# usnistgov/thermoextrap

Measured on AMD Instinct MI355X. Metric: samples/s for order-4 comoment bootstrap (N_samp x N_obs x nrep resample_vals), higher is better.
Workload: dtype f64; 1 GPU; north: central-comoment bootstrap, N_samp=1e+08, N_obs=32, order=4, nrep=1000, exact multinomial device sampler; n_samp=100000000, n_obs=32, order=4, nrep=1000, parallelism=state-points x1

## Files before the change

thermoextrap_amd/csrc/txm_i8g.h:

```cpp
#pragma once
#include "txm_i8t_common.h"

namespace txm {

constexpr int G_REPS = 128;
constexpr int G_KSTEP_BYTES = 32 * G_REPS;
constexpr int G_TILE_BYTES = SM_T * G_REPS;

static inline size_t count_table_bytes(int64_t ntiles, int64_t nreps) {
  return (size_t)cdiv(nreps, G_REPS) * (size_t)ntiles * G_TILE_BYTES;
}

constexpr int G_BS = 4;
constexpr int G_RAW = 2 * G_BS * 256;
#ifndef TXM_G_LEAD
#define TXM_G_LEAD 2
#endif
constexpr uint32_t G_LEAD = TXM_G_LEAD;

__device__ __forceinline__ void g_dma16(const void *sbase, uint32_t voff, uint32_t lds_dst) {
#ifdef TXM_G_NO_DMA
  return;
#endif
  asm volatile("s_mov_b32 m0, %2\n\ts_nop 0\n\tglobal_load_lds_dwordx4 %1, %0" ::"s"(sbase), "v"(voff), "s"(lds_dst) : "memory", "m0");
}
__device__ __forceinline__ void g_dma16_stream(const void *sbase, uint32_t voff, uint32_t lds_dst) {
#ifdef TXM_G_NO_DMA
  return;
#endif
#ifdef TXM_G_TABLE_PLAIN
  asm volatile("s_mov_b32 m0, %2\n\ts_nop 0\n\tglobal_load_lds_dwordx4 %1, %0" ::"s"(sbase), "v"(voff), "s"(lds_dst) : "memory", "m0");
#else
  asm volatile("s_mov_b32 m0, %2\n\ts_nop 0\n\tglobal_load_lds_dwordx4 %1, %0 nt" ::"s"(sbase), "v"(voff), "s"(lds_dst) : "memory", "m0");
#endif
}
__device__ __forceinline__ void g_dma4(const void *sbase, uint32_t voff, uint32_t lds_dst) {
#ifdef TXM_G_NO_DMA
  return;
#endif
  asm volatile("s_mov_b32 m0, %2\n\ts_nop 0\n\tglobal_load_lds_dword %1, %0" ::"s"(sbase), "v"(voff), "s"(lds_dst) : "memory", "m0");
}
__device__ __forceinline__ void g_load16(v4i &dst, const void *sbase, uint32_t voff) {
  asm volatile("global_load_dwordx4 %0, %1, %2" : "=v"(dst) : "v"(voff), "s"(sbase) : "memory");
}
typedef uint32_t g_v16u __attribute__((ext_vector_type(16)));
__device__ __forceinline__ uint32_t g_min_progress(const uint32_t *pg) {
  g_v16u v;
  asm volatile("s_load_dwordx16 %0, %1, 0x0 glc\n\ts_waitcnt lgkmcnt(0)" : "=s"(v) : "s"(pg) : "memory");
  uint32_t m = 0xffffffffu;
#pragma unroll
  for (int i = 0; i < 16; ++i) {
    const uint32_t e = v[i] == 0u ? 0xffffffffu : v[i];
    m = e < m ? e : m;
  }
  return m;
}
__device__ __forceinline__ uint32_t g_lane_now() {
  uint32_t l;
  asm volatile("v_mbcnt_lo_u32_b32 %0, -1, 0\n\tv_mbcnt_hi_u32_b32 %0, -1, %0" : "=v"(l));
  return l;
}
template <int N>
__device__ __forceinline__ void g_wait_vm() {
  asm volatile("s_waitcnt vmcnt(%0)" ::"n"(N) : "memory");
}


int launch_count_table(const uint32_t *counts, int64_t nrep, int64_t N, uint32_t k0, uint32_t k1, uint32_t rep_base,
                       int64_t rep_begin, int64_t n_groups, unsigned char *table, hipStream_t st);

bool i8g_applicable(const double *x, int64_t ldx_s, int64_t C, const double *y, int64_t ldy_s);
int launch_resample_i8g(const I8Args &a, int K, bool weighted, const unsigned char *table, int64_t rep_begin, int n_grp,
                        hipStream_t st);

bool i8gn_applicable(const double *x, int64_t ldx_s, int64_t C, int K);
int launch_resample_i8gn(const I8Args &a, int K, bool weighted, const unsigned char *table, int64_t rep_begin, int n_grp,
                         size_t table_state_stride, hipStream_t st);

}
```

thermoextrap_amd/csrc/txm_resample_i8g.hip:

```cpp
#include "txm_i8g.h"

namespace txm {

constexpr int G_XR = 4;
static_assert(G_XR == G_BS && G_BS == 4, "the wait counts below are written for blocks of four k-steps");
constexpr int G_XRB = 8;
constexpr int G_FU = 2176;

#ifdef TXM_G_FOUR_QUARTERS
template <int NS> constexpr int G_QUARTERS = 4;
#elif defined(TXM_G_SIX_QUARTERS)
template <int NS> constexpr int G_QUARTERS = NS == 1 ? 8 : NS == 2 ? 6 : 4;
#else
template <int NS> constexpr int G_QUARTERS = NS == 1 ? 8 : 4;
#endif

template <int J0, int JN, bool WEIGHTED, bool YS>
constexpr int G_NQ = (J0 == 0 && JN == 1 && WEIGHTED && YS) ? 4 : G_QUARTERS<JN + (YS ? 1 : 0)>;

template <int J0, int JN, bool WEIGHTED, bool YS>
__global__ __launch_bounds__(T_BLOCK) __attribute__((amdgpu_waves_per_eu(2, 2))) void resample_i8g_kernel(
    const I8Args a, const int K, const unsigned char *__restrict__ table, const int64_t rep_begin, const int n_grp) {
  constexpr int NS = JN + (YS ? 1 : 0);
  static_assert(JN >= 1 && NS <= 3 && J0 + JN <= 8, "row sets");
  constexpr int NPT = JN + ((YS && WEIGHTED && J0 > 0) ? 1 : 0);
  constexpr int NX = YS ? 2 : 1;
  constexpr int WREG = NS * T_PB;
  constexpr int NQ = G_NQ<J0, JN, WEIGHTED, YS>;
  constexpr int A_STEP = NQ * 1024;
  constexpr int PPW = G_BS * NQ / T_WAVES;
  static_assert(G_BS * NQ % T_WAVES == 0, "count pieces per wave");
  constexpr int OFF_A = T_WAVES * WREG;
  constexpr bool XBLK = !YS;
#ifdef TXM_G_ADIR
  constexpr bool ADIR = XBLK && NS == 2;
#else
  constexpr bool ADIR = false;
#endif
  constexpr int XRN = XBLK ? G_XRB : G_XR;
  constexpr int OFF_X = OFF_A + 2 * G_BS * A_STEP;
  constexpr int OFF_Y = OFF_X + T_WAVES * XRN * 1024;
  constexpr int OFF_RAW = OFF_Y + (YS ? T_WAVES * XRN * 1024 : 0);
  constexpr int OFF_F = OFF_RAW + 3 * G_RAW;
  constexpr int OFF_FS = OFF_F + 3 * 2 * G_FU;
  static_assert(G_BS * 16 * NPT * 8 <= G_FU, "factor lines");
  extern __shared__ __attribute__((aligned(16))) unsigned char lds[];
  uint32_t *fsum = reinterpret_cast<uint32_t *>(lds + OFF_FS);

  const int wave = __builtin_amdgcn_readfirstlane((int)(threadIdx.x >> 6)), lane = threadIdx.x & 63;
  const int n32 = lane & 31, half = lane >> 5;
  const uint32_t wreg = (uint32_t)(wave * WREG);

  const int b = blockIdx.x;
  const int n_wgg = (4 * n_grp + NQ - 1) / NQ;
  const int64_t win = (int64_t)((b >> 3) / n_wgg) * 8 + (b & 7);
  const int grp = (b >> 3) % n_wgg;
  if (win >= a.nwin) return;
  if (a.wflag[win] != 0u) return;
  const int64_t rep0 = rep_begin + (int64_t)grp * (32 * NQ);
  const int64_t WT = a.win_tiles;
  const int64_t t0 = win * WT;
  const int64_t t1 = t0 + WT < a.ntiles ? t0 + WT : a.ntiles;
  const int nsteps = (int)(t1 - t0) * T_STEPS;
  const int nblk = nsteps / G_BS;
  const unsigned char *tab = table + (size_t)t0 * G_TILE_BYTES;
  auto q_off = [&](int Q) -> size_t {
    int gq = grp * NQ + Q;
    if (gq >= 4 * n_grp) gq = grp * NQ;
    return (size_t)(gq >> 2) * (size_t)a.ntiles * G_TILE_BYTES + (size_t)(gq & 3) * 1024;
  };

  const int ps = lane >> 2, cl = lane & 3;
  const int col = 4 * wave + cl;
  const int ccol = col < a.C ? col : 0;
  const int qsrc = 4 * wave < a.C ? wave : 0;
  const uint32_t rd_off = wreg + (uint32_t)(((lane >> 4) & 1) * (T_PLANE + 128) + (16 * half + ((lane & 15) >> 1)) * 16 + (lane & 1) * 8);
  const int tcl = (n32 >> 2) & 3, tdg = 4 * (n32 >> 4) + (n32 & 3);
  const int ofi = wave >> 1;
  const int odig = 4 * (wave & 1) + cl;
  const uint32_t osel = odig < 7 ? (((uint32_t)odig << 24) | 0x000c0c0cu) : 0x0c0c0c0cu;
  const uint32_t oxor = odig < 6 ? 0x80000000u : 0u;

  const double *wt = a.wtab + win * I8_WT_STRIDE;
  const double pu = a.pivot[0];
  const double inv_du = wt[I8_WT_INVDU];
  const double inv_w = WEIGHTED ? wt[I8_WT_INVW] : 1.0;
  const double sc = wt[I8_WT_SC + ccol];
  const double px = a.pivot[1 + a.col0 + ccol];
  const double *wty = YS ? a.ywtab + win * I8_WT_STRIDE : wt;
  const double scy = YS ? wty[I8_WT_SC + ccol] : 0.0;
  const double py = YS ? a.ypivot[1 + a.col0 + ccol] : 0.0;

  v16i acc[NS][NQ];
#pragma unroll
  for (int e = 0; e < NS; ++e)
#pragma unroll
    for (int q = 0; q < NQ; ++q) acc[e][q] = (v16i)(0);

#ifdef TXM_G_CLOCKS
  const long long gc0 = clock64(), gr0 = wall_clock64();
#endif
#ifdef TXM_G_TIMING
  long long tm[8] = {0, 0, 0, 0, 0, 0, 0, 0};
  long long tk0 = clock64();
#define G_TICK(k) do { const long long t1_ = clock64(); tm[k] += t1_ - tk0; tk0 = t1_; } while (0)
#else
#define G_TICK(k) do {} while (0)
#endif
  auto chunk_sample = [&](int c) -> int64_t {
    int64_t b0 = (t0 + (c >> 5)) * SM_T;
    if (b0 > a.N - SM_T) b0 = a.N - SM_T;
    return b0 + 32 * (c & 31);
  };
  const uint32_t xring = (uint32_t)(OFF_X + wave * XRN * 1024), yring = (uint32_t)(OFF_Y + wave * XRN * 1024);
  int cq = 0;
  const char *xq = reinterpret_cast<const char *>(a.x + chunk_sample(0) * a.ldx_s);
  const char *yq = YS ? reinterpret_cast<const char *>(a.y + chunk_sample(0) * a.ldy_s) : nullptr;
  const int64_t xstep = 32 * a.ldx_s * 8, ystep = YS ? 32 * a.ldy_s * 8 : 0;
  const bool loader = !XBLK || wave < 4;
  const int qsrc2 = 4 * (wave + 4) < a.C ? wave + 4 : 0;
  const int64_t xcol1 = (a.col0 + 4 * qsrc) * 8, xcol2 = (a.col0 + 4 * qsrc2) * 8;
  size_t qoff[NQ];
#pragma unroll
  for (int Q = 0; Q < NQ; ++Q) qoff[Q] = q_off(Q);
  auto x_request = [&](int slot) {
#ifdef TXM_G_NO_XDMA
    if (slot >= 0) { ++cq; return; }
#endif
    if constexpr (XBLK) {
      if (loader) {
        const uint32_t ln = g_lane_now();
        const uint32_t row = (ln >> 1) * (uint32_t)(a.ldx_s * 8) + (ln & 1) * 16u + (uint32_t)(a.col0 * 8);
        g_dma16(xq, row + (uint32_t)(32 * qsrc), xring + (uint32_t)slot * 1024u);
        g_dma16(xq, row + (uint32_t)(32 * qsrc2), xring + (uint32_t)(4 * XRN * 1024) + (uint32_t)slot * 1024u);
      }
    } else {
      const uint32_t ln = g_lane_now();
      const uint32_t cb = (ln & 1) * 16u + (uint32_t)((a.col0 + 4 * qsrc) * 8);
      g_dma16(xq, (ln >> 1) * (uint32_t)(a.ldx_s * 8) + cb, xring + (uint32_t)slot * 1024u);
      if constexpr (YS) g_dma16(yq, (ln >> 1) * (uint32_t)(a.ldy_s * 8) + cb, yring + (uint32_t)slot * 1024u);
    }
    ++cq;
    if (cq < nsteps) {
      if ((cq & 31) == 0) {
        const int64_t i0 = chunk_sample(cq);
        xq = reinterpret_cast<const char *>(a.x + i0 * a.ldx_s);
        if constexpr (YS) yq = reinterpret_cast<const char *>(a.y + i0 * a.ldy_s);
      } else {
        xq += xstep;
        if constexpr (YS) yq += ystep;
      }
    }
  };
  auto a_request = [&](int B, int piece = -1) {
    const int Bc = B < nblk ? B : nblk - 1;
#ifdef TXM_G_NO_ADMA
    if (Bc >= 0) return;
#endif
    if constexpr (XBLK) {
      if (!loader) return;
      const unsigned char *src = tab + (size_t)(Bc * G_BS + wave) * G_KSTEP_BYTES;
      const uint32_t dst = (uint32_t)(OFF_A + (B & 1) * (G_BS * A_STEP) + wave * A_STEP);
#pragma unroll
      for (int Q = 0; Q < NQ; ++Q)
        if (piece < 0 || piece == Q) g_dma16_stream(src + q_off(Q), g_lane_now() * 16u, dst + (uint32_t)(Q * 1024));
    } else {
      const uint32_t l16 = g_lane_now() * 16u;
#pragma unroll
      for (int k = 0; k < PPW; ++k) {
        const int i = wave * PPW + k, st = i / NQ, Q = i % NQ;
        g_dma16_stream(tab + (size_t)(Bc * G_BS + st) * G_KSTEP_BYTES + q_off(Q), l16,
                (uint32_t)(OFF_A + (B & 1) * (G_BS * A_STEP) + st * A_STEP + Q * 1024));
      }
    }
  };
  auto raw_request = [&](int B) {
    int c = B * G_BS + 1 + (wave & 3);
    if (c > nsteps - 1) c = nsteps - 1;
    if constexpr (XBLK) {
      if (!loader) return;
      const int64_t i0 = chunk_sample(c);
      const uint32_t l4 = g_lane_now() * 4u;
      g_dma4(a.u + i0, l4, (uint32_t)(OFF_RAW + (B % 3) * G_RAW + wave * 256));
      if constexpr (WEIGHTED) g_dma4(a.w + i0, l4, (uint32_t)(OFF_RAW + (B % 3) * G_RAW + G_BS * 256 + wave * 256));
    } else {
      const double *src = ((WEIGHTED && wave >= 4) ? a.w : a.u) + chunk_sample(c);
      g_dma4(src, g_lane_now() * 4u, (uint32_t)(OFF_RAW + (B % 3) * G_RAW + (wave >> 2) * (G_BS * 256) + (wave & 3) * 256));
    }
  };
  auto stage_factors = [&](int B) {
#ifndef TXM_G_SW
#define TXM_G_SW 6
#endif
    constexpr int SW = TXM_G_SW;
    if (wave < SW || wave >= SW + 2) return;
    const int e = (int)g_lane_now() + (wave - SW) * 64;
    const double *raw = reinterpret_cast<const double *>(lds + OFF_RAW + (B % 3) * G_RAW);
#ifdef TXM_G_TIMING
    G_TICK(1);
    double r0 = raw[e];
    asm volatile("s_waitcnt lgkmcnt(0)" : "+v"(r0));
    G_TICK(5);
    const double du = (r0 - pu) * inv_du;
#else
    const double du = (raw[e] - pu) * inv_du;
#endif
    double pw = WEIGHTED ? raw[G_BS * 32 + e] * inv_w : 1.0;
    double *f = reinterpret_cast<double *>(lds + OFF_F + (B % 3) * (2 * G_FU) + ((e >> 4) & 1) * G_FU) + (((e >> 5) * 16 + (e & 15)) * NPT);
    if constexpr (NPT > JN) f[JN] = pw;
#pragma unroll
    for (int k = 0; k < J0; ++k) pw *= du;
#pragma unroll
    for (int jj = 0; jj < JN; ++jj) {
      if (WEIGHTED || J0 + jj > 0) f[jj] = pw;
      pw *= du;
    }
  };

  auto store_x2 = [&](uint32_t lo0, uint32_t hi0, uint32_t lo1, uint32_t hi1, int off) {
#ifdef TXM_G_PLAIN_STORES
    typedef __attribute__((address_space(3))) uint32_t *lds_u32;
    const uint32_t base = wreg + g_lane_now() * 4u;
    *(lds_u32)(lds + base + off) = lo0;
    *(lds_u32)(lds + base + off + T_PLANE + 128) = hi0;
    *(lds_u32)(lds + base + off + 256) = lo1;
    *(lds_u32)(lds + base + off + 256 + T_PLANE + 128) = hi1;
    return;
#endif
#ifdef TXM_G_PLAIN_STORES_ASM
    {
      const uint32_t base = wreg + g_lane_now() * 4u + (uint32_t)off;
      asm volatile("ds_write2st64_b32 %0, %1, %2 offset0:0 offset1:1\n\t"
                   "ds_write2st64_b32 %3, %4, %5 offset0:0 offset1:1"
                   :
                   : "v"(base), "v"(lo0), "v"(lo1), "v"(base + (uint32_t)(T_PLANE + 128)), "v"(hi0), "v"(hi1)
                   : "memory");
      return;
    }
#endif
    asm volatile("s_mov_b32 m0, %4\n\ts_nop 0\n\t"
                 "ds_write_addtid_b32 %0 offset:%5\n\t"
                 "ds_write_addtid_b32 %1 offset:%6\n\t"
                 "ds_write_addtid_b32 %2 offset:%7\n\t"
                 "ds_write_addtid_b32 %3 offset:%8"
                 :
                 : "v"(lo0), "v"(hi0), "v"(lo1), "v"(hi1), "s"(wreg), "n"(off), "n"(off + T_PLANE + 128), "n"(off + 256),
                   "n"(off + 256 + T_PLANE + 128)
                 : "memory", "m0");
  };
  auto produce_row = [&](auto fic, double (&f)[2], const double (&d)[2], auto &&ahead) {
    constexpr int fi = decltype(fic)::value;
    uint32_t lo[2], hi[2];
#pragma unroll
    for (int uu = 0; uu < 2; ++uu) {
      const uint64_t bits = (uint64_t)__double_as_longlong(fma(f[uu], d[uu], T_MAGIC));
      lo[uu] = (uint32_t)bits ^ 0x80808080u;
      hi[uu] = (uint32_t)(bits >> 32) ^ 0x00008080u;
    }
#ifdef TXM_G_NO_OVERLAY
    if (false) {
#else
    if (fi < JN && ofi == fi) {
#endif
#pragma unroll
      for (int uu = 0; uu < 2; ++uu) {
        const uint64_t ub = (uint64_t)__double_as_longlong(__builtin_ldexp(f[uu], 50) + T_MAGIC);
        uint32_t dig;
        asm volatile("v_perm_b32 %0, %1, %2, %3" : "=v"(dig) : "v"((uint32_t)(ub >> 32)), "v"((uint32_t)ub), "v"(osel));
        hi[uu] = (hi[uu] & 0x00ffffffu) | (dig ^ oxor);
      }
    }
    ahead();
    store_x2(lo[0], hi[0], lo[1], hi[1], fi * T_PB);
  };

  typedef __attribute__((address_space(3))) const double *lds_cd;
  typedef __attribute__((address_space(3))) const v4i *lds_cv4;

  if (threadIdx.x < 32 * NQ) {
    const int64_t r = rep0 + threadIdx.x;
    uint32_t s = 0;
    if (r < a.nrep)
      for (int64_t t = t0; t < t1; ++t) s += a.counts[(size_t)r * a.ntiles + t];
    fsum[threadIdx.x] = s;
  }
  for (int e = threadIdx.x; e < T_WAVES * WREG / 16; e += T_BLOCK) reinterpret_cast<uint4 *>(lds)[e] = make_uint4(0, 0, 0, 0);
  double d_du[2], d_w[2] = {1.0, 1.0};
  {
    const int64_t i0 = chunk_sample(0);
#pragma unroll
    for (int uu = 0; uu < 2; ++uu) {
      d_du[uu] = (a.u[i0 + 16 * uu + ps] - pu) * inv_du;
      if constexpr (WEIGHTED) d_w[uu] = a.w[i0 + 16 * uu + ps] * inv_w;
    }
  }
  asm volatile("s_waitcnt vmcnt(0)" ::: "memory");
  raw_request(0);
  raw_request(1);
  if constexpr (!ADIR) a_request(0);
  if constexpr (XBLK) {
    x_request(7);
#pragma unroll
    for (int c = 0; c < G_BS; ++c) x_request(c);
  } else {
#pragma unroll
    for (int c = 0; c < G_XR; ++c) x_request(c);
  }
  v4i AD[
#ifdef TXM_G_ADIR
      (XBLK && NS == 2) ? G_BS : 1
#else
      1
#endif
  ][NQ];
#ifdef TXM_G_ADIR
  if constexpr (XBLK && NS == 2) {
    const uint32_t l16 = g_lane_now() * 16u;
#pragma unroll
    for (int pp = 0; pp < G_BS; ++pp)
#pragma unroll
      for (int q = 0; q < NQ; ++q) g_load16(AD[pp][q], tab + (size_t)pp * G_KSTEP_BYTES + qoff[q], l16);
  }
#endif
  asm volatile("s_waitcnt vmcnt(0) lgkmcnt(0)\n\ts_barrier" ::: "memory");
  stage_factors(0);
  {
    const uint32_t xa = xring + (uint32_t)(ps * 32 + cl * 8) + (XBLK ? 7u * 1024u : 0u);
    double dx[2], dy[2] = {0.0, 0.0};
#pragma unroll
    for (int uu = 0; uu < 2; ++uu) {
      dx[uu] = (*(lds_cd)(lds + xa + uu * 512) - px) * sc;
      if constexpr (YS) dy[uu] = (*(lds_cd)(lds + xa + (yring - xring) + uu * 512) - py) * scy;
    }
    t_static_for<NS>([&](auto fic) {
      constexpr int fi = decltype(fic)::value;
      double f[2];
#pragma unroll
      for (int uu = 0; uu < 2; ++uu) {
        if constexpr (YS && fi == JN) {
          f[uu] = WEIGHTED ? d_w[uu] : 1.0;
        } else {
          double pw = WEIGHTED ? d_w[uu] : 1.0;
          for (int q = 0; q < J0 + fi; ++q) pw *= d_du[uu];
          f[uu] = pw;
        }
      }
      if constexpr (YS && fi == JN) produce_row(fic, f, dy, [] {});
      else produce_row(fic, f, dx, [] {});
    });
  }
  asm volatile("s_waitcnt lgkmcnt(0)\n\ts_barrier" ::: "memory");
  if constexpr (!XBLK) x_request(0);
  G_TICK(0);

  uint32_t *pg = a.progress != nullptr ? a.progress + (size_t)win * 16 : nullptr;
#ifdef TXM_G_PRIO
  if (wave >= 4) __builtin_amdgcn_s_setprio(TXM_G_PRIO);
#endif
  auto read_factors = [&](auto pnc, auto finc, uint32_t fb, double (&f)[2]) {
    constexpr int pn = decltype(pnc)::value, fin = decltype(finc)::value;
#pragma unroll
    for (int uu = 0; uu < 2; ++uu) {
      if constexpr (YS && fin == JN) {
        if constexpr (WEIGHTED) f[uu] = *(lds_cd)(lds + fb + uu * G_FU + (pn * 16 * NPT + (J0 == 0 ? 0 : JN)) * 8);
        else f[uu] = 1.0;
      } else if constexpr (!WEIGHTED && J0 == 0 && fin == 0) {
        f[uu] = 1.0;
      } else {
        f[uu] = *(lds_cd)(lds + fb + uu * G_FU + (pn * 16 * NPT + fin) * 8);
      }
    }
  };
  v4i A[NQ];
  constexpr bool BT2 = NS >= 2;
  v2i Bt[BT2 ? 2 : 1][2];
  double f[2], xr[2], yr[2] = {0.0, 0.0};
  uint32_t f_va = (uint32_t)(OFF_F + ps * NPT * 8);
  uint32_t x_va = xring + (uint32_t)(ps * 32 + cl * 8);
  {
    const uint32_t a_va0 = (uint32_t)OFF_A + (uint32_t)lane * 16u;
#pragma unroll
    for (int q = 0; q < NQ; ++q) {
      if constexpr (!ADIR) A[q] = *(lds_cv4)(lds + a_va0 + q * 1024);
    }
    Bt[0][0] = T_TRREAD((lds_v2i)(lds + rd_off));
    Bt[0][1] = T_TRREAD((lds_v2i)(lds + rd_off + 128));
    read_factors(std::integral_constant<int, 0>{}, std::integral_constant<int, 0>{}, f_va, f);
#pragma unroll
    for (int uu = 0; uu < 2; ++uu) xr[uu] = *(lds_cd)(lds + x_va + (XBLK ? 0 : 1024) + uu * 512);
  }
#pragma unroll 1
  for (int B = 0; B < nblk; ++B) {
    if (pg != nullptr && wave == 0 && (B & 7) == 0) {
      const uint32_t done = (uint32_t)(B >> 3) + 1u;
      if (lane == 0) __hip_atomic_store(&pg[grp & 15], done, __ATOMIC_RELAXED, __HIP_MEMORY_SCOPE_AGENT);
#pragma unroll 1
      for (int spin = 0; spin < I8_THROTTLE_SPINS; ++spin) {
        if (done <= g_min_progress(pg) + G_LEAD) break;
        __builtin_amdgcn_s_sleep(32);
      }
    }
    G_TICK(1);
    stage_factors(B + 1);
    G_TICK(7);
    raw_request(B + 2);
    const unsigned char *blk_asrc = nullptr;
    uint32_t blk_adst = 0, blk_l16 = 0, blk_xrow = 0;
    if constexpr (XBLK) {
      if (loader) {
        const int Bn = B + 1 < nblk ? B + 1 : nblk - 1;
        blk_asrc = tab + (size_t)(Bn * G_BS + wave) * G_KSTEP_BYTES;
        blk_adst = (uint32_t)(OFF_A + ((B + 1) & 1) * (G_BS * A_STEP) + wave * A_STEP);
        const uint32_t ln = g_lane_now();
        blk_l16 = ln * 16u;
        blk_xrow = (ln >> 1) * (uint32_t)(a.ldx_s * 8) + (ln & 1) * 16u;
      }
    }
    auto a_piece = [&](int Q) {
#ifndef TXM_G_NO_ADMA
      if constexpr (!ADIR)
        if (loader) g_dma16_stream(blk_asrc + qoff[Q], blk_l16, blk_adst + (uint32_t)(Q * 1024));
#endif
    };
    const unsigned char *nb_src = nullptr;
    uint32_t nb_l16 = 0;
    if constexpr (ADIR) {
      const int Bn = B + 1 < nblk ? B + 1 : nblk - 1;
      nb_src = tab + (size_t)(Bn * G_BS) * G_KSTEP_BYTES;
      nb_l16 = g_lane_now() * 16u;
    }
    auto x_chunk = [&](int i) {
#ifndef TXM_G_NO_XDMA
      if (loader) {
        const uint32_t dst = xring + (uint32_t)((4 * ((B + 1) & 1) + i) * 1024);
        g_dma16(xq + xcol1, blk_xrow, dst);
        g_dma16(xq + xcol2, blk_xrow, dst + (uint32_t)(4 * XRN * 1024));
      }
#endif
      ++cq;
      if (cq < nsteps) {
        if ((cq & 31) == 0) xq = reinterpret_cast<const char *>(a.x + chunk_sample(cq) * a.ldx_s);
        else xq += xstep;
      }
    };
#ifdef TXM_G_BURST
    constexpr bool SPREAD = false;
#else
    constexpr bool SPREAD = XBLK && NS >= 2;
#endif
    if constexpr (!SPREAD) {
      if constexpr (XBLK) {
#pragma unroll
        for (int Q = 0; Q < NQ; ++Q) a_piece(Q);
#pragma unroll
        for (int i = 0; i < G_BS; ++i) x_chunk(i);
      } else {
        a_request(B + 1);
      }
    }
    constexpr int ISSUE_SLOTS = 2 * NS;
    auto issue_items = [&](auto kc) {
      constexpr int k = decltype(kc)::value;
      if constexpr (SPREAD && k < ISSUE_SLOTS) {
        if constexpr (ADIR) {
          static_assert(!ADIR || ISSUE_SLOTS == G_BS, "one x chunk a slot");
          x_chunk(k);
        } else {
#pragma unroll
          for (int j = 0; j < NQ + 4; ++j)
            if (j * ISSUE_SLOTS / (NQ + 4) == k) {
              if (j < 8 && (j & 1) == 0) a_piece(j >> 1);
              else if (j < 8) x_chunk(j >> 1);
              else a_piece(j - 4);
            }
        }
      }
    };
    G_TICK(2);
    uint32_t a_va = (uint32_t)(OFF_A + (B & 1) * (G_BS * A_STEP)) + (uint32_t)lane * 16u;
    asm volatile("" : "+v"(f_va), "+v"(x_va), "+v"(a_va));
#ifdef TXM_G_NO_PIN
#define G_PIN() do {} while (0)
#else
#define G_PIN() __builtin_amdgcn_sched_barrier(0)
#endif
    t_static_for<G_BS>([&](auto pc) {
      constexpr int p = decltype(pc)::value;
      double dx[2], dy[2] = {0.0, 0.0};
      if constexpr (ADIR) {
        constexpr int R = WEIGHTED ? 2 : 1;
        constexpr int NL = 12 + (p < 2 ? 4 : 8) + R;
        G_PIN();
        if (loader) asm volatile("s_waitcnt vmcnt(%0)" ::"n"(NL) : "memory");
        else asm volatile("s_waitcnt vmcnt(12)" ::: "memory");
        G_PIN();
      }
      t_static_for<NS>([&](auto fic) {
        constexpr int fi = decltype(fic)::value;
        constexpr bool last = fi == NS - 1;
        if constexpr (p == G_BS - 1 && last) {
          G_TICK(3);
          if constexpr (ADIR) {
            if (loader) asm volatile("s_waitcnt vmcnt(7) lgkmcnt(0)" ::: "memory");
            else asm volatile("s_waitcnt lgkmcnt(0)" ::: "memory");
          } else {
            asm volatile("s_waitcnt vmcnt(%0) lgkmcnt(0)" ::"n"(XBLK ? 0 : 3 * NX) : "memory");
          }
#ifndef TXM_G_NO_BARRIER
          asm volatile("s_barrier" ::: "memory");
#endif
          G_TICK(6);
        }
        auto ahead = [&]() {
          if constexpr (!last) {
            read_factors(pc, std::integral_constant<int, fi + 1>{}, f_va, f);
          } else if constexpr (p < G_BS - 1) {
            read_factors(std::integral_constant<int, p + 1>{}, std::integral_constant<int, 0>{}, f_va, f);
          } else {
            f_va = (uint32_t)(OFF_F + ((B + 1) % 3) * (2 * G_FU) + ps * NPT * 8);
            asm volatile("" : "+v"(f_va));
            read_factors(std::integral_constant<int, 0>{}, std::integral_constant<int, 0>{}, f_va, f);
          }
          if constexpr (YS && fi == JN - 1) {
#pragma unroll
            for (int uu = 0; uu < 2; ++uu) yr[uu] = *(lds_cd)(lds + x_va + (OFF_Y - OFF_X) + ((p + 1) & 3) * 1024 + uu * 512);
          }
          if constexpr (last) {
            if constexpr (XBLK) {
              if constexpr (p == G_BS - 1) {
                x_va = xring + (uint32_t)(ps * 32 + cl * 8) + (uint32_t)(((B + 1) & 1) * 4096);
                asm volatile("" : "+v"(x_va));
              }
#pragma unroll
              for (int uu = 0; uu < 2; ++uu) xr[uu] = *(lds_cd)(lds + x_va + (p == G_BS - 1 ? 0 : p + 1) * 1024 + uu * 512);
            } else {
              g_wait_vm<2 * NX + (p == G_BS - 1 ? 0 : PPW + 1)>();
#pragma unroll
              for (int uu = 0; uu < 2; ++uu) xr[uu] = *(lds_cd)(lds + x_va + ((p + 2) & 3) * 1024 + uu * 512);
            }
          }
        };
        constexpr int bcur = BT2 ? ((p * NS + fi) & 1) : 0;
        const v4i Bv = {Bt[bcur][0][0], Bt[bcur][0][1], Bt[bcur][1][0], Bt[bcur][1][1]};
        auto mfma_q = [&](auto qc) {
          constexpr int q = decltype(qc)::value;
          if constexpr (ADIR) t_mfma<true>(acc[fi][q], AD[p][q], Bv);
          else t_mfma<true>(acc[fi][q], A[q], Bv);
#ifndef TXM_G_NO_AREAD
          if constexpr (last && ADIR) {
            g_load16(AD[p][q], nb_src + (size_t)p * G_KSTEP_BYTES + qoff[q], nb_l16);
          } else if constexpr (last) {
            if constexpr (p == G_BS - 1) {
              const uint32_t a_vn = (uint32_t)(OFF_A + ((B + 1) & 1) * (G_BS * A_STEP)) + g_lane_now() * 16u;
              A[q] = *(lds_cv4)(lds + a_vn + q * 1024);
            } else {
              A[q] = *(lds_cv4)(lds + a_va + (p + 1) * A_STEP + q * 1024);
            }
          }
#endif
        };
        G_PIN();
        t_static_for<(0 + 1) * NQ / 4 - 0 * NQ / 4>([&](auto jc) { mfma_q(std::integral_constant<int, 0 * NQ / 4 + decltype(jc)::value>{}); });
        G_PIN();
        issue_items(std::integral_constant<int, p * NS + fi>{});
        if constexpr (BT2) {
          constexpr int fn = (fi + 1) % NS;
          Bt[bcur ^ 1][0] = T_TRREAD((lds_v2i)(lds + rd_off + fn * T_PB));
          Bt[bcur ^ 1][1] = T_TRREAD((lds_v2i)(lds + rd_off + fn * T_PB + 128));
        }
        G_PIN();
        if constexpr (fi == 0) {
#pragma unroll
          for (int uu = 0; uu < 2; ++uu) dx[uu] = (xr[uu] - px) * sc;
        }
        if constexpr (YS && fi == JN) {
#pragma unroll
          for (int uu = 0; uu < 2; ++uu) dy[uu] = (yr[uu] - py) * scy;
        }
        uint32_t lo[2], hi[2];
#pragma unroll
        for (int uu = 0; uu < 2; ++uu) {
#ifdef TXM_G_NO_SLICE
          lo[uu] = 0x01020304u + uu;
          hi[uu] = 0x04030201u + uu;
          asm volatile("" : "+v"(lo[uu]), "+v"(hi[uu]));
#else
          const double dd = (YS && fi == JN) ? dy[uu] : dx[uu];
          const uint64_t bits = (uint64_t)__double_as_longlong(fma(f[uu], dd, T_MAGIC));
          lo[uu] = (uint32_t)bits;
          hi[uu] = (uint32_t)(bits >> 32);
#endif
        }
        G_PIN();
        t_static_for<(1 + 1) * NQ / 4 - 1 * NQ / 4>([&](auto jc) { mfma_q(std::integral_constant<int, 1 * NQ / 4 + decltype(jc)::value>{}); });
        G_PIN();
#ifndef TXM_G_NO_SLICE
#pragma unroll
        for (int uu = 0; uu < 2; ++uu) {
          lo[uu] ^= 0x80808080u;
          hi[uu] ^= 0x00008080u;
        }
#endif
        G_PIN();
#if !defined(TXM_G_NO_OVERLAY) && !defined(TXM_G_NO_SLICE)
        if (fi < JN && ofi == fi) {
#ifdef TXM_G_OVERLAY_RECOMPUTE
          const uint32_t od_l = 4u * (uint32_t)(wave & 1) + (g_lane_now() & 3u);
          const uint32_t osel_l = od_l < 7u ? ((od_l << 24) | 0x000c0c0cu) : 0x0c0c0c0cu;
          const uint32_t oxor_l = od_l < 6u ? 0x80000000u : 0u;
#else
          const uint32_t osel_l = osel, oxor_l = oxor;
#endif
#pragma unroll
          for (int uu = 0; uu < 2; ++uu) {
            const uint64_t ub = (uint64_t)__double_as_longlong(__builtin_ldexp(f[uu], 50) + T_MAGIC);
            uint32_t dig;
            asm volatile("v_perm_b32 %0, %1, %2, %3" : "=v"(dig) : "v"((uint32_t)(ub >> 32)), "v"((uint32_t)ub), "v"(osel_l));
            hi[uu] = (hi[uu] & 0x00ffffffu) | (dig ^ oxor_l);
          }
        }
#endif
        G_PIN();
#ifndef TXM_G_NO_AHEAD
        ahead();
#endif
        G_PIN();
        t_static_for<(2 + 1) * NQ / 4 - 2 * NQ / 4>([&](auto jc) { mfma_q(std::integral_constant<int, 2 * NQ / 4 + decltype(jc)::value>{}); });
        G_PIN();
#ifndef TXM_G_NO_PRODUCE
        store_x2(lo[0], hi[0], lo[1], hi[1], fi * T_PB);
#else
        asm volatile("" ::"v"(lo[0]), "v"(hi[0]), "v"(lo[1]), "v"(hi[1]));
#endif
        G_PIN();
        t_static_for<(3 + 1) * NQ / 4 - 3 * NQ / 4>([&](auto jc) { mfma_q(std::integral_constant<int, 3 * NQ / 4 + decltype(jc)::value>{}); });
        G_PIN();
#ifndef TXM_G_NO_TRREAD
        if constexpr (!BT2) {
          Bt[0][0] = T_TRREAD((lds_v2i)(lds + rd_off));
          Bt[0][1] = T_TRREAD((lds_v2i)(lds + rd_off + 128));
        }
#endif
        G_PIN();
      });
      if constexpr (!XBLK) x_request((p + 1) & 3);
    });
  }

  constexpr int XS = 65, XT = 16 * XS;
  static_assert(OFF_A + T_WAVES * XT * 4 <= OFF_RAW, "flush scratch inside the count and x rings");
  asm volatile("s_waitcnt vmcnt(0) lgkmcnt(0)\n\ts_barrier" ::: "memory");
  if (pg != nullptr && threadIdx.x == 0) __hip_atomic_store(&pg[grp & 15], 0xfffffff0u, __ATOMIC_RELAXED, __HIP_MEMORY_SCOPE_AGENT);
  auto odig_of = [](int w, int c) { return 4 * (w & 1) + c; };
  uint32_t *xw = reinterpret_cast<uint32_t *>(lds + OFF_A) + wave * XT;
  auto flush_tile = [&](v16i &T, int q, int rs) {
    uint32_t z = 0;
    asm volatile("" : "+v"(z));
    const int64_t opq = (int64_t)z;
    const bool is_y = YS && rs == JN;
    if (is_y) {
      const int64_t rrow = rep0 + 32 * q + 4 * half;
      const int c = 4 * wave + tcl;
      const bool valid = tdg < I8_NSL && c < a.C;
      const int dgt = tdg < I8_NSL ? tdg : 0;
      double dsc = wty[I8_WT_DSP + 0] * wty[I8_WT_DSC + (c < a.C ? c : 0)];
      double *base = a.part_y + (((size_t)win * a.nrep_pad + rrow) * 8 + dgt) * a.cpad + c + opq;
      const size_t stride = (size_t)8 * a.cpad;
      dsc *= (double)((int64_t)1 << (8 * dgt));
      const int bias = dgt == I8_NSL - 1 ? T_D6_BIAS : 0;
      if (valid) {
#pragma unroll
        for (int r = 0; r < 16; ++r) {
          const int m = (r >> 2) * 8 + (r & 3);
          if (rrow + m < a.nrep) {
            const int v = T[r] - bias * (int)fsum[32 * q + m + 4 * half];
            base[(size_t)m * stride] = (double)v * dsc;
          }
        }
      }
      return;
    }
#pragma unroll
    for (int r = 0; r < 16; ++r) xw[r * XS + lane] = (uint32_t)T[r];
    const int j = J0 + rs;
#pragma unroll
    for (int i = 0; i < 2; ++i) {
      const int o = lane + 64 * i, m = o >> 2, q4 = o & 3;
      const int rr = ((m >> 3) << 2) | (m & 3), hh = (m >> 2) & 1;
      const int64_t rrow = rep0 + 32 * q + m;
      if (rrow < a.nrep) {
        const uint32_t *src = xw + rr * XS + 32 * hh + 4 * q4;
        const int fs = (int)fsum[32 * q + m];
        const int c = 4 * wave + q4;
        if (c < a.C) {
          int v[I8_NSL];
#pragma unroll
          for (int d = 0; d < I8_NSL; ++d) v[d] = (int)src[16 * (d >> 2) + (d & 3)];
          v[I8_NSL - 1] -= T_D6_BIAS * fs;
          const double dsc0 = wt[I8_WT_DSP + j] * wt[I8_WT_DSC + c];
          double sum = 0.0;
#pragma unroll
          for (int d = 0; d < I8_NSL; ++d) {
            double pd = (double)v[d] * (dsc0 * (double)((int64_t)1 << (8 * d)));
            asm volatile("" : "+v"(pd));
            sum = d == 0 ? pd : sum + pd;
          }
          a.part_x[(((size_t)win * a.nrep_pad + rrow) * K + j) * a.cpad + c + opq] = sum;
        }
        const int dgt = odig_of(wave, q4);
        if (ofi == rs && dgt < 7) {
          const int v7 = (int)src[16 + 3] - (dgt == I8_NSL - 1 ? T_D6_BIAS * fs : 0);
          const double dsc = (wt[I8_WT_DSP + j] * 0x1p-50) * (double)((int64_t)1 << (8 * dgt));
          a.part_u[((size_t)win * a.nrep_pad + rrow) * K * 8 + (size_t)j * 8 + dgt + opq] = (double)v7 * dsc;
        }
      }
    }
  };
#pragma unroll
  for (int fi = 0; fi < NS; ++fi)
#pragma unroll
    for (int q = 0; q < NQ; ++q) flush_tile(acc[fi][q], q, fi);
#ifdef TXM_G_CLOCKS
  if (lane == 0 && (blockIdx.x == 0 || blockIdx.x == 1064)) {
    double *o = a.wtab + a.nwin * I8_WT_STRIDE + ((blockIdx.x ? 1 : 0) * T_WAVES + wave) * 8;
    o[0] = (double)(clock64() - gc0);
    o[1] = (double)(wall_clock64() - gr0);
  }
#endif
#ifdef TXM_G_TIMING
  G_TICK(0);
  if (lane == 0 && (blockIdx.x == 0 || blockIdx.x == 1064))
    for (int k = 0; k < 8; ++k) a.wtab[a.nwin * I8_WT_STRIDE + ((blockIdx.x ? 1 : 0) * T_WAVES + wave) * 8 + k] = (double)tm[k];
#endif
}

template <int J0, int JN, bool WEIGHTED, bool YS>
static int launch_pass_g(const I8Args &a, int K, const unsigned char *table, int64_t rep_begin, int n_grp, hipStream_t st) {
  constexpr int NS = JN + (YS ? 1 : 0);
  constexpr int NQ = G_NQ<J0, JN, WEIGHTED, YS>;
  const size_t lds = (size_t)T_WAVES * NS * T_PB + 2 * G_BS * NQ * 1024 + (size_t)(YS ? 2 * G_XR : G_XRB) * T_WAVES * 1024 + 3 * G_RAW +
                     3 * 2 * G_FU + 32 * NQ * sizeof(uint32_t);
  const dim3 grid((unsigned)(cdiv(a.nwin, 8) * 8 * cdiv(4 * (int64_t)n_grp, NQ)));
  if (a.progress != nullptr) TXM_HIP(hipMemsetAsync(a.progress, 0, (size_t)cdiv(a.nwin, 8) * 8 * 16 * sizeof(uint32_t), st));
  TXM_SET_MAX_LDS((&resample_i8g_kernel<J0, JN, WEIGHTED, YS>), lds);
  hipLaunchKernelGGL((resample_i8g_kernel<J0, JN, WEIGHTED, YS>), grid, dim3(T_BLOCK), lds, st, a, K, table, rep_begin, n_grp);
  TXM_LAUNCH_CHECK();
  return TXM_OK;
}

bool i8g_applicable(const double *x, int64_t ldx_s, int64_t C, const double *y, int64_t ldy_s) {
  if (C <= 16) return false;
  const int64_t cq = (C + 3) / 4 * 4;
  if (((uintptr_t)x & 15) != 0 || (ldx_s & 1) != 0 || cq > ldx_s) return false;
  if (y != nullptr && (((uintptr_t)y & 15) != 0 || (ldy_s & 1) != 0 || cq > ldy_s)) return false;
  return true;
}

int launch_resample_i8g(const I8Args &a, int K, bool weighted, const unsigned char *table, int64_t rep_begin, int n_grp,
                        hipStream_t st) {
  const bool ys = a.y != nullptr;
  const int rows = K + (ys ? 1 : 0), np = (rows + 2) / 3;
#ifdef TXM_G_EVEN_SPLIT
  const bool greedy = false;
#else
  const bool greedy = !ys && rows > 3 && rows % 3 == 1;
#endif
  int j0 = 0;
  for (int i = 0; i < np; ++i) {
    const int n = greedy ? (i < np - 1 ? 3 : 1) : rows / np + (i < rows % np ? 1 : 0);
    const bool last = i == np - 1;
    const int jn = n - ((last && ys) ? 1 : 0);
    const bool y_here = last && ys;
    int rc = TXM_ERR_INVALID;
#define G_CASE(J0_, JN_)                                                                                         \
  if (j0 == J0_ && jn == JN_) {                                                                                  \
    if (y_here) {                                                                                                \
      if constexpr (JN_ <= 2) rc = weighted ? launch_pass_g<J0_, JN_, true, true>(a, K, table, rep_begin, n_grp, st) \
                                            : launch_pass_g<J0_, JN_, false, true>(a, K, table, rep_begin, n_grp, st); \
    } else rc = weighted ? launch_pass_g<J0_, JN_, true, false>(a, K, table, rep_begin, n_grp, st)                \
                       : launch_pass_g<J0_, JN_, false, false>(a, K, table, rep_begin, n_grp, st);              \
  }
#ifdef TXM_G_ONLY03
    if (j0 == 0 && jn == 3 && !y_here && !weighted) rc = launch_pass_g<0, 3, false, false>(a, K, table, rep_begin, n_grp, st);
#elif defined(TXM_G_ONLY32)
    if (j0 == 3 && jn == 2 && !y_here && !weighted) rc = launch_pass_g<3, 2, false, false>(a, K, table, rep_begin, n_grp, st);
#elif defined(TXM_G_ONLY02)
    if (j0 == 0 && jn == 2 && !y_here && !weighted) rc = launch_pass_g<0, 2, false, false>(a, K, table, rep_begin, n_grp, st);
#elif defined(TXM_G_ONLY01)
    if (j0 == 0 && jn == 1 && !y_here && !weighted) rc = launch_pass_g<0, 1, false, false>(a, K, table, rep_begin, n_grp, st);
#else
    G_CASE(0, 1) G_CASE(0, 2) G_CASE(0, 3) G_CASE(2, 1) G_CASE(2, 2) G_CASE(3, 1) G_CASE(3, 2) G_CASE(3, 3)
    G_CASE(5, 1) G_CASE(5, 2) G_CASE(6, 1) G_CASE(6, 2)
#endif
#undef G_CASE
    if (rc != TXM_OK) {
      if (rc == TXM_ERR_INVALID) set_error("resample_i8g: no pass for powers %d..%d", j0, j0 + jn - 1);
      return rc;
    }
    j0 += jn;
  }
  return TXM_OK;
}

}
```

Before: 623.1 million samples/s.

## Add twelve-wave i8g kernel for three-row passes sharing count tiles across row sets

Adds a new 768-thread (twelve-wave) variant of the i8g resample kernel, used for passes with three power rows and no y. Each wave takes one (row-set, quarter) pair, so a single block covers all three powers and four rep quarters. The count table and x tiles are loaded once by four loader waves and shared, where previously this work ran across more blocks. This cuts redundant table and x traffic and changes occupancy to three waves per EU. In exchange it uses a large LDS footprint and a hand-tuned schedule with new wait and barrier placements.

After: 525.8 million samples/s. -15.6%, worse.

```diff
diff --git a/thermoextrap_amd/csrc/txm_i8g.h b/thermoextrap_amd/csrc/txm_i8g.h
--- a/thermoextrap_amd/csrc/txm_i8g.h
+++ b/thermoextrap_amd/csrc/txm_i8g.h
@@ -17,6 +17,10 @@
 #define TXM_G_LEAD 2
 #endif
 constexpr uint32_t G_LEAD = TXM_G_LEAD;
+constexpr int G3_WAVES = 12;
+constexpr int G3_BLOCK = 64 * G3_WAVES;
+constexpr int G3_XSLOT = 32 * 32 * 8;
+constexpr int G3_XRN = 8;
 
 __device__ __forceinline__ void g_dma16(const void *sbase, uint32_t voff, uint32_t lds_dst) {
 #ifdef TXM_G_NO_DMA
diff --git a/thermoextrap_amd/csrc/txm_resample_i8g.hip b/thermoextrap_amd/csrc/txm_resample_i8g.hip
--- a/thermoextrap_amd/csrc/txm_resample_i8g.hip
+++ b/thermoextrap_amd/csrc/txm_resample_i8g.hip
@@ -734,6 +734,378 @@
 #endif
 }
 
+constexpr int G3_WREG = 2 * T_PB;
+constexpr int G3_OFF_A = G3_WAVES * G3_WREG;
+constexpr int G3_OFF_X = G3_OFF_A + 2 * G_BS * 4 * 1024;
+constexpr int G3_OFF_RAW = G3_OFF_X + G3_XRN * G3_XSLOT;
+constexpr int G3_OFF_F = G3_OFF_RAW + 2 * G_RAW;
+constexpr int G3_OFF_PS = G3_OFF_F + 2 * 2 * G_FU;
+constexpr int G3_OFF_FS = G3_OFF_PS + 32 * 16;
+constexpr int G3_LDS = G3_OFF_FS + 128 * 4;
+static_assert(G3_LDS <= 163840, "LDS of the twelve-wave instance");
+static_assert((G3_OFF_X & 63) == 0 && (G3_XSLOT & 63) == 0, "x-ring addresses: quad 1 = quad 0 ^ 32");
+
+template <int J0, bool WEIGHTED>
+__global__ __launch_bounds__(G3_BLOCK) __attribute__((amdgpu_waves_per_eu(3, 3))) void resample_i8g_kernel_w12(
+    const I8Args a, const int K, const unsigned char *__restrict__ table, const int64_t rep_begin, const int n_grp) {
+  constexpr int JN = 3, NQ = 4, NPT = JN, A_STEP = NQ * 1024;
+  static_assert(G_BS * 16 * NPT * 8 <= G_FU, "factor lines");
+  extern __shared__ __attribute__((aligned(16))) unsigned char lds[];
+  uint32_t *fsum = reinterpret_cast<uint32_t *>(lds + G3_OFF_FS);
+
+  const int wave = __builtin_amdgcn_readfirstlane((int)(threadIdx.x >> 6)), lane = threadIdx.x & 63;
+  const int half = (lane & 63) >> 5;
+  const int rs = wave >> 2, kq = wave & 3;
+  const bool loader = wave < 4;
+  const bool ovl = kq == rs;
+  const uint32_t wreg = (uint32_t)(wave * G3_WREG);
+
+  const int b = blockIdx.x;
+  const int n_wgg = n_grp;
+  const int64_t win = (int64_t)((b >> 3) / n_wgg) * 8 + (b & 7);
+  const int grp = (b >> 3) % n_wgg;
+  if (win >= a.nwin) return;
+  if (a.wflag[win] != 0u) return;
+  const int64_t rep0 = rep_begin + (int64_t)grp * (32 * NQ);
+  const int64_t WT = a.win_tiles;
+  const int64_t t0 = win * WT;
+  const int64_t t1 = t0 + WT < a.ntiles ? t0 + WT : a.ntiles;
+  const int nsteps = (int)(t1 - t0) * T_STEPS;
+  const int nblk = nsteps / G_BS;
+  const unsigned char *tab = table + (size_t)t0 * G_TILE_BYTES + (size_t)grp * (size_t)a.ntiles * G_TILE_BYTES;
+
+  const int ps = lane >> 2, cl = lane & 3;
+  const uint32_t rd_off = wreg + (uint32_t)(((lane >> 4) & 1) * (T_PLANE + 128) + (16 * half + ((lane & 15) >> 1)) * 16 + (lane & 1) * 8);
+
+  const double *wt = a.wtab + win * I8_WT_STRIDE;
+  const double pu = a.pivot[0];
+  const double inv_du = wt[I8_WT_INVDU];
+  const double inv_w = WEIGHTED ? wt[I8_WT_INVW] : 1.0;
+
+  v16i acc[2][NQ];
+#pragma unroll
+  for (int h = 0; h < 2; ++h)
+#pragma unroll
+    for (int q = 0; q < NQ; ++q) acc[h][q] = (v16i)(0);
+
+  auto chunk_sample = [&](int c) -> int64_t {
+    int64_t b0 = (t0 + (c >> 5)) * SM_T;
+    if (b0 > a.N - SM_T) b0 = a.N - SM_T;
+    return b0 + 32 * (c & 31);
+  };
+  int cq = 0;
+  const char *xq = reinterpret_cast<const char *>(a.x + chunk_sample(0) * a.ldx_s + a.col0);
+  const int64_t xstep = 32 * a.ldx_s * 8;
+  auto x_voff = [&](int j) -> uint32_t {
+    const uint32_t ln = g_lane_now();
+    const uint32_t row = (uint32_t)(4 * j) + (ln >> 4);
+    uint32_t sc = (ln & 15u) ^ ((2u * row) & 15u);
+    if (4 * (int)(sc >> 1) >= a.C) sc &= 1u;
+    return row * (uint32_t)(a.ldx_s * 8) + sc * 16u;
+  };
+  auto x_chunk = [&](int slot, uint32_t v0, uint32_t v1) {
+    if (loader) {
+      const uint32_t dst = (uint32_t)(G3_OFF_X + slot * G3_XSLOT + wave * 2048);
+      g_dma16(xq, v0, dst);
+      g_dma16(xq, v1, dst + 1024u);
+    }
+    ++cq;
+    if (cq < nsteps) {
+      if ((cq & 31) == 0) xq = reinterpret_cast<const char *>(a.x + chunk_sample(cq) * a.ldx_s + a.col0);
+      else xq += xstep;
+    }
+  };
+  auto a_piece = [&](int B, int Q) {
+    if (!loader) return;
+    const int Bc = B < nblk ? B : nblk - 1;
+    g_dma16_stream(tab + (size_t)(Bc * G_BS + wave) * G_KSTEP_BYTES + Q * 1024, g_lane_now() * 16u,
+                   (uint32_t)(G3_OFF_A + (B & 1) * (G_BS * A_STEP) + wave * A_STEP + Q * 1024));
+  };
+  auto raw_request = [&](int B) {
+    if (!loader) return;
+    int c = B * G_BS + 1 + wave;
+    if (c > nsteps - 1) c = nsteps - 1;
+    const int64_t i0 = chunk_sample(c);
+    const uint32_t l4 = g_lane_now() * 4u;
+    g_dma4(a.u + i0, l4, (uint32_t)(G3_OFF_RAW + (B & 1) * G_RAW + wave * 256));
+    if constexpr (WEIGHTED) g_dma4(a.w + i0, l4, (uint32_t)(G3_OFF_RAW + (B & 1) * G_RAW + G_BS * 256 + wave * 256));
+  };
+  auto stage_factors = [&](int B) {
+    if (wave != 7 && wave != 11) return;
+    const int e = (int)g_lane_now() + (wave == 7 ? 0 : 64);
+    const double *raw = reinterpret_cast<const double *>(lds + G3_OFF_RAW + (B & 1) * G_RAW);
+    const double du = (raw[e] - pu) * inv_du;
+    double pw = WEIGHTED ? raw[G_BS * 32 + e] * inv_w : 1.0;
+    double *f = reinterpret_cast<double *>(lds + G3_OFF_F + (B & 1) * (2 * G_FU) + ((e >> 4) & 1) * G_FU) + (((e >> 5) * 16 + (e & 15)) * NPT);
+#pragma unroll
+    for (int k = 0; k < J0; ++k) pw *= du;
+#pragma unroll
+    for (int jj = 0; jj < JN; ++jj) {
+      if (WEIGHTED || J0 + jj > 0) f[jj] = pw;
+      pw *= du;
+    }
+  };
+  auto store_x2 = [&](uint32_t lo0, uint32_t hi0, uint32_t lo1, uint32_t hi1, int off) {
+    asm volatile("s_mov_b32 m0, %4\n\ts_nop 0\n\t"
+                 "ds_write_addtid_b32 %0 offset:%5\n\t"
+                 "ds_write_addtid_b32 %1 offset:%6\n\t"
+                 "ds_write_addtid_b32 %2 offset:%7\n\t"
+                 "ds_write_addtid_b32 %3 offset:%8"
+                 :
+                 : "v"(lo0), "v"(hi0), "v"(lo1), "v"(hi1), "s"(wreg), "n"(off), "n"(off + T_PLANE + 128), "n"(off + 256),
+                   "n"(off + 256 + T_PLANE + 128)
+                 : "memory", "m0");
+  };
+  typedef __attribute__((address_space(3))) const double *lds_cd;
+  typedef __attribute__((address_space(3))) const v4i *lds_cv4;
+  typedef double v2d __attribute__((ext_vector_type(2)));
+  typedef __attribute__((address_space(3))) const v2d *lds_cv2d;
+  auto make_words = [&](auto hc, const double (&xr)[2], v2d pxs, const double (&f)[2]) {
+    constexpr int h = decltype(hc)::value;
+    uint32_t lo[2], hi[2];
+#pragma unroll
+    for (int uu = 0; uu < 2; ++uu) {
+      const double dx = (xr[uu] - pxs[0]) * pxs[1];
+      const uint64_t bits = (uint64_t)__double_as_longlong(fma(f[uu], dx, T_MAGIC));
+      lo[uu] = (uint32_t)bits ^ 0x80808080u;
+      hi[uu] = (uint32_t)(bits >> 32) ^ 0x00008080u;
+    }
+    if (ovl) {
+      const uint32_t od = 4u * h + (g_lane_now() & 3u);
+      const uint32_t osel = od < 7u ? ((od << 24) | 0x000c0c0cu) : 0x0c0c0c0cu;
+      const uint32_t oxor = od < 6u ? 0x80000000u : 0u;
+#pragma unroll
+      for (int uu = 0; uu < 2; ++uu) {
+        double fo = f[uu];
+        asm volatile("" : "+v"(fo));
+        const uint64_t ub = (uint64_t)__double_as_longlong(__builtin_ldexp(fo, 50) + T_MAGIC);
+        uint32_t dig;
+        asm volatile("v_perm_b32 %0, %1, %2, %3" : "=v"(dig) : "v"((uint32_t)(ub >> 32)), "v"((uint32_t)ub), "v"(osel));
+        hi[uu] = (hi[uu] & 0x00ffffffu) | (dig ^ oxor);
+      }
+    }
+    store_x2(lo[0], hi[0], lo[1], hi[1], h * T_PB);
+  };
+
+  if (threadIdx.x < 32 * NQ) {
+    const int64_t r = rep0 + threadIdx.x;
+    uint32_t s = 0;
+    if (r < a.nrep)
+      for (int64_t t = t0; t < t1; ++t) s += a.counts[(size_t)r * a.ntiles + t];
+    fsum[threadIdx.x] = s;
+  } else if (threadIdx.x >= 256 && threadIdx.x < 256 + 32) {
+    const int c = threadIdx.x - 256, cc = c < a.C ? c : 0;
+    double *o = reinterpret_cast<double *>(lds + G3_OFF_PS) + 2 * c;
+    o[0] = a.pivot[1 + a.col0 + cc];
+    o[1] = wt[I8_WT_SC + cc];
+  }
+  for (int e = threadIdx.x; e < G3_WAVES * G3_WREG / 16; e += G3_BLOCK) reinterpret_cast<uint4 *>(lds)[e] = make_uint4(0, 0, 0, 0);
+  double d_du[2], d_w[2] = {1.0, 1.0};
+  {
+    const int64_t i0 = chunk_sample(0);
+#pragma unroll
+    for (int uu = 0; uu < 2; ++uu) {
+      d_du[uu] = (a.u[i0 + 16 * uu + ps] - pu) * inv_du;
+      if constexpr (WEIGHTED) d_w[uu] = a.w[i0 + 16 * uu + ps] * inv_w;
+    }
+  }
+  asm volatile("s_waitcnt vmcnt(0)" ::: "memory");
+  raw_request(0);
+  raw_request(1);
+#pragma unroll
+  for (int Q = 0; Q < NQ; ++Q) a_piece(0, Q);
+  {
+    const uint32_t v0 = x_voff(2 * wave), v1 = x_voff(2 * wave + 1);
+    x_chunk(7, v0, v1);
+#pragma unroll
+    for (int c = 0; c < G_BS; ++c) x_chunk(c, v0, v1);
+  }
+  asm volatile("s_waitcnt vmcnt(0) lgkmcnt(0)\n\ts_barrier" ::: "memory");
+  stage_factors(0);
+  const uint32_t x_l = (uint32_t)(ps * 256 + (((4 * kq + (cl >> 1)) ^ ((2 * ps) & 15)) * 16) + (cl & 1) * 8);
+  const uint32_t ps_l = (uint32_t)(G3_OFF_PS + (8 * kq + cl) * 16);
+  {
+    double f[2];
+#pragma unroll
+    for (int uu = 0; uu < 2; ++uu) {
+      double pw = WEIGHTED ? d_w[uu] : 1.0;
+      for (int q = 0; q < J0 + rs; ++q) pw *= d_du[uu];
+      f[uu] = pw;
+    }
+    t_static_for<2>([&](auto hc) {
+      constexpr int h = decltype(hc)::value;
+      const uint32_t xa = (uint32_t)(G3_OFF_X + 7 * G3_XSLOT) + (x_l ^ (32u * h));
+      double xr[2];
+#pragma unroll
+      for (int uu = 0; uu < 2; ++uu) xr[uu] = *(lds_cd)(lds + xa + uu * 4096);
+      const v2d pxs = *(lds_cv2d)(lds + ps_l + h * 64);
+      make_words(hc, xr, pxs, f);
+    });
+  }
+  asm volatile("s_waitcnt lgkmcnt(0)\n\ts_barrier" ::: "memory");
+
+  uint32_t *pg = a.progress != nullptr ? a.progress + (size_t)win * 16 : nullptr;
+  const bool unit_f = !WEIGHTED && J0 == 0 && rs == 0;
+  const uint32_t a_l = (uint32_t)G3_OFF_A + (uint32_t)lane * 16u;
+  const uint32_t f_l = (uint32_t)(G3_OFF_F + (ps * NPT + rs) * 8);
+  const uint32_t x_l0 = (uint32_t)G3_OFF_X + x_l, x_l1 = x_l0 ^ 32u;
+  v4i Ab[2], Bq[2];
+  Ab[0] = *(lds_cv4)(lds + a_l);
+#pragma unroll
+  for (int h = 0; h < 2; ++h) {
+    const v2i b0 = T_TRREAD((lds_v2i)(lds + rd_off + h * T_PB)), b1 = T_TRREAD((lds_v2i)(lds + rd_off + h * T_PB + 128));
+    Bq[h] = (v4i){b0[0], b0[1], b1[0], b1[1]};
+  }
+#pragma unroll 1
+  for (int B2 = 0; B2 < nblk; B2 += 2) {
+    t_static_for<2>([&](auto parc) {
+      constexpr int par = decltype(parc)::value;
+      const int B = B2 + par;
+      if (pg != nullptr && wave == 0 && (B & 7) == 0) {
+        const uint32_t done = (uint32_t)(B >> 3) + 1u;
+        if (lane == 0) __hip_atomic_store(&pg[grp & 15], done, __ATOMIC_RELAXED, __HIP_MEMORY_SCOPE_AGENT);
+#pragma unroll 1
+        for (int spin = 0; spin < I8_THROTTLE_SPINS; ++spin) {
+          if (done <= g_min_progress(pg) + G_LEAD) break;
+          __builtin_amdgcn_s_sleep(32);
+        }
+      }
+      stage_factors(B + 1);
+      raw_request(B + 2);
+      t_static_for<G_BS>([&](auto pc) {
+        constexpr int p = decltype(pc)::value;
+        constexpr int AO = par * (G_BS * A_STEP) + p * A_STEP;
+        constexpr int XO = (4 * par + p) * G3_XSLOT;
+        constexpr int FO = par * (2 * G_FU) + p * 16 * NPT * 8;
+        double f[2], xr[2];
+        v2d pxs;
+        G_PIN();
+#pragma unroll
+        for (int uu = 0; uu < 2; ++uu) {
+          f[uu] = unit_f ? 1.0 : *(lds_cd)(lds + f_l + FO + uu * G_FU);
+          xr[uu] = *(lds_cd)(lds + x_l0 + XO + uu * 4096);
+        }
+        pxs = *(lds_cv2d)(lds + ps_l);
+        Ab[1] = *(lds_cv4)(lds + a_l + AO + 1024);
+        G_PIN();
+        t_mfma<true>(acc[0][0], Ab[0], Bq[0]);
+        G_PIN();
+        t_mfma<true>(acc[1][0], Ab[0], Bq[1]);
+        G_PIN();
+        make_words(std::integral_constant<int, 0>{}, xr, pxs, f);
+        G_PIN();
+        Ab[0] = *(lds_cv4)(lds + a_l + AO + 2048);
+#pragma unroll
+        for (int uu = 0; uu < 2; ++uu) xr[uu] = *(lds_cd)(lds + x_l1 + XO + uu * 4096);
+        pxs = *(lds_cv2d)(lds + ps_l + 64);
+        G_PIN();
+        t_mfma<true>(acc[0][1], Ab[1], Bq[0]);
+        G_PIN();
+        t_mfma<true>(acc[1][1], Ab[1], Bq[1]);
+        G_PIN();
+        Ab[1] = *(lds_cv4)(lds + a_l + AO + 3072);
+        G_PIN();
+        t_mfma<true>(acc[0][2], Ab[0], Bq[0]);
+        G_PIN();
+        make_words(std::integral_constant<int, 1>{}, xr, pxs, f);
+        G_PIN();
+        t_mfma<true>(acc[1][2], Ab[0], Bq[1]);
+        G_PIN();
+        if constexpr (p == G_BS - 1) {
+          asm volatile("s_waitcnt vmcnt(0) lgkmcnt(0)\n\ts_barrier" ::: "memory");
+          Ab[0] = *(lds_cv4)(lds + a_l + (1 - par) * (G_BS * A_STEP));
+        } else {
+          Ab[0] = *(lds_cv4)(lds + a_l + AO + A_STEP);
+        }
+        G_PIN();
+        t_mfma<true>(acc[0][3], Ab[1], Bq[0]);
+        G_PIN();
+        {
+          const v2i b0 = T_TRREAD((lds_v2i)(lds + rd_off)), b1 = T_TRREAD((lds_v2i)(lds + rd_off + 128));
+          Bq[0] = (v4i){b0[0], b0[1], b1[0], b1[1]};
+        }
+        G_PIN();
+        t_mfma<true>(acc[1][3], Ab[1], Bq[1]);
+        G_PIN();
+        {
+          const v2i b0 = T_TRREAD((lds_v2i)(lds + rd_off + T_PB)), b1 = T_TRREAD((lds_v2i)(lds + rd_off + T_PB + 128));
+          Bq[1] = (v4i){b0[0], b0[1], b1[0], b1[1]};
+        }
+        G_PIN();
+        if constexpr (p < 2) {
+          const uint32_t v0 = x_voff(2 * wave), v1 = x_voff(2 * wave + 1);
+#pragma unroll
+          for (int i = 2 * p; i < 2 * p + 2; ++i) {
+            a_piece(B + 1, i);
+            x_chunk(4 * (1 - par) + i, v0, v1);
+          }
+        }
+        G_PIN();
+      });
+    });
+  }
+
+  constexpr int XS = 65, XT = 16 * XS;
+  static_assert(G3_OFF_A + G3_WAVES * XT * 4 <= G3_OFF_RAW, "flush scratch inside the count and x rings");
+  asm volatile("s_waitcnt vmcnt(0) lgkmcnt(0)\n\ts_barrier" ::: "memory");
+  if (pg != nullptr && threadIdx.x == 0) __hip_atomic_store(&pg[grp & 15], 0xfffffff0u, __ATOMIC_RELAXED, __HIP_MEMORY_SCOPE_AGENT);
+  uint32_t *xw = reinterpret_cast<uint32_t *>(lds + G3_OFF_A) + wave * XT;
+  const int j = J0 + rs;
+  auto flush_tile = [&](v16i &T, int q, int qd) {
+    uint32_t z = 0;
+    asm volatile("" : "+v"(z));
+    const int64_t opq = (int64_t)z;
+#pragma unroll
+    for (int r = 0; r < 16; ++r) xw[r * XS + lane] = (uint32_t)T[r];
+#pragma unroll
+    for (int i = 0; i < 2; ++i) {
+      const int o = lane + 64 * i, m = o >> 2, q4 = o & 3;
+      const int rr = ((m >> 3) << 2) | (m & 3), hh = (m >> 2) & 1;
+      const int64_t rrow = rep0 + 32 * q + m;
+      if (rrow < a.nrep) {
+        const uint32_t *src = xw + rr * XS + 32 * hh + 4 * q4;
+        const int fs = (int)fsum[32 * q + m];
+        const int c = 4 * qd + q4;
+        if (c < a.C) {
+          int v[I8_NSL];
+#pragma unroll
+          for (int d = 0; d < I8_NSL; ++d) v[d] = (int)src[16 * (d >> 2) + (d & 3)];
+          v[I8_NSL - 1] -= T_D6_BIAS * fs;
+          const double dsc0 = wt[I8_WT_DSP + j] * wt[I8_WT_DSC + c];
+          double sum = 0.0;
+#pragma unroll
+          for (int d = 0; d < I8_NSL; ++d) {
+            double pd = (double)v[d] * (dsc0 * (double)((int64_t)1 << (8 * d)));
+            asm volatile("" : "+v"(pd));
+            sum = d == 0 ? pd : sum + pd;
+          }
+          a.part_x[(((size_t)win * a.nrep_pad + rrow) * K + j) * a.cpad + c + opq] = sum;
+        }
+        const int dgt = 4 * (qd & 1) + q4;
+        if (ovl && dgt < 7) {
+          const int v7 = (int)src[16 + 3] - (dgt == I8_NSL - 1 ? T_D6_BIAS * fs : 0);
+          const double dsc = (wt[I8_WT_DSP + j] * 0x1p-50) * (double)((int64_t)1 << (8 * dgt));
+          a.part_u[((size_t)win * a.nrep_pad + rrow) * K * 8 + (size_t)j * 8 + dgt + opq] = (double)v7 * dsc;
+        }
+      }
+    }
+  };
+#pragma unroll
+  for (int h = 0; h < 2; ++h)
+#pragma unroll
+    for (int q = 0; q < NQ; ++q) flush_tile(acc[h][q], q, 2 * kq + h);
+}
+
+template <int J0, bool WEIGHTED>
+static int launch_pass_g3w(const I8Args &a, int K, const unsigned char *table, int64_t rep_begin, int n_grp, hipStream_t st) {
+  const dim3 grid((unsigned)(cdiv(a.nwin, 8) * 8 * (int64_t)n_grp));
+  if (a.progress != nullptr) TXM_HIP(hipMemsetAsync(a.progress, 0, (size_t)cdiv(a.nwin, 8) * 8 * 16 * sizeof(uint32_t), st));
+  TXM_SET_MAX_LDS((&resample_i8g_kernel_w12<J0, WEIGHTED>), G3_LDS);
+  hipLaunchKernelGGL((resample_i8g_kernel_w12<J0, WEIGHTED>), grid, dim3(G3_BLOCK), G3_LDS, st, a, K, table, rep_begin, n_grp);
+  TXM_LAUNCH_CHECK();
+  return TXM_OK;
+}
+
 template <int J0, int JN, bool WEIGHTED, bool YS>
 static int launch_pass_g(const I8Args &a, int K, const unsigned char *table, int64_t rep_begin, int n_grp, hipStream_t st) {
   constexpr int NS = JN + (YS ? 1 : 0);
@@ -777,7 +1149,9 @@
     if (y_here) {                                                                                                \
       if constexpr (JN_ <= 2) rc = weighted ? launch_pass_g<J0_, JN_, true, true>(a, K, table, rep_begin, n_grp, st) \
                                             : launch_pass_g<J0_, JN_, false, true>(a, K, table, rep_begin, n_grp, st); \
-    } else rc = weighted ? launch_pass_g<J0_, JN_, true, false>(a, K, table, rep_begin, n_grp, st)                \
+    } else if constexpr (JN_ == 3) rc = weighted ? launch_pass_g3w<J0_, true>(a, K, table, rep_begin, n_grp, st)  \
+                                                 : launch_pass_g3w<J0_, false>(a, K, table, rep_begin, n_grp, st); \
+    else rc = weighted ? launch_pass_g<J0_, JN_, true, false>(a, K, table, rep_begin, n_grp, st)                  \
                        : launch_pass_g<J0_, JN_, false, false>(a, K, table, rep_begin, n_grp, st);              \
   }
 #ifdef TXM_G_ONLY03
```
